# ChrisTho23/DrakeGPT

Measured on NVIDIA B200. Metric: train_tokens_per_sec_TransformerLM_scaled, higher is better.
Workload: dtype bf16

## Files before the change

drakegpt_b200/csrc/attn_tc.cu:

```cuda
#include <cuda.h>
#include <stdlib.h>

#include "common.cuh"
#include "ptx.cuh"

namespace dgpt {

using namespace ptx;

int make_tmap_bf16_2d(CUtensorMap* map, const void* base, int64_t inner, int64_t outer, int64_t ld, int box_outer);

static constexpr int HD = 64;
static constexpr int QT = 128;
static constexpr float kLog2e = 1.4426950408889634f;

struct AttnTcP {
  void *o, *dq, *dk, *dv;
  const void *o_in, *d_o;
  float* lse;
  int64_t o_rs, dq_rs, dk_rs, dv_rs, do_rs;
  int B, NH, T;
  float scale, inv_keep;
  uint32_t thr, site;
  uint64_t seed;
// ... 447 lines not shown
#pragma unroll
      for (int cc = 0; cc < HD; cc += 32) {
        uint32_t r[32];
        tmem_ld32(taddr + nkv * 64 + cc, r);
        tmem_ld_wait();
#pragma unroll
        for (int j = 0; j < 4; ++j) {
          uint4 w;
          w.x = pack_bf16(__uint_as_float(r[8 * j]) * oscale, __uint_as_float(r[8 * j + 1]) * oscale);
          w.y = pack_bf16(__uint_as_float(r[8 * j + 2]) * oscale, __uint_as_float(r[8 * j + 3]) * oscale);
          w.z = pack_bf16(__uint_as_float(r[8 * j + 4]) * oscale, __uint_as_float(r[8 * j + 5]) * oscale);
          w.w = pack_bf16(__uint_as_float(r[8 * j + 6]) * oscale, __uint_as_float(r[8 * j + 7]) * oscale);
          *reinterpret_cast<uint4*>(orow + cc + 8 * j) = w;
        }
      }
      tc_fence_before();
      __syncwarp();
      if (lane == 0) mbar_arrive(&slot_free[g]);
      FTS(5);
    }
  }
  tc_fence_before();
  __syncthreads();
  if (warp == 9) {
    tc_fence_after();
    tmem_dealloc<512>(tmem);
  }
  clock_probe_end(sc.probe);
}

static constexpr int kFwd3Threads = 576;
static constexpr int kFwd3Smem = 2 * kFwd2QK + 2 * 32768 + 4096 + 256 + 1024;

__global__ void __launch_bounds__(kFwd3Threads, 1)
attn_fwd_tc3_kernel(const __grid_constant__ CUtensorMap map_q32, const __grid_constant__ CUtensorMap map_k,
                    const __grid_constant__ CUtensorMap map_v, AttnTcP p, FwdSched sc) {
  extern __shared__ uint8_t smem_raw[];
  uint8_t* smem = reinterpret_cast<uint8_t*>((reinterpret_cast<uintptr_t>(smem_raw) + 1023) & ~(uintptr_t)1023);
  uint8_t* sQK = smem;
  uint8_t* sV = smem + 2 * kFwd2QK;
  float* xch = reinterpret_cast<float*>(sV + 2 * 32768);
  uint64_t* bars = reinterpret_cast<uint64_t*>(sV + 2 * 32768 + 4096);
  uint64_t *qk_full = bars, *qk_empty = bars + 2, *v_full = bars + 4, *v_empty = bars + 6, *s_full = bars + 8,
           *p_full = bars + 10, *o_full = bars + 12, *slot_free = bars + 14;
  uint32_t* tmem_slot = reinterpret_cast<uint32_t*>(bars + 16);

  clock_probe_begin(sc.probe);
  const int warp = threadIdx.x >> 5, lane = threadIdx.x & 31;
  const int ntile = p.T / QT;

  const int G = gridDim.x, c = blockIdx.x;
  const int hq = sc.nheavy / G, hr = sc.nheavy % G;
  const int nh_c = hq + (c < hr ? 1 : 0);
  const int U = (kWHeavy * sc.nheavy + kWLight * sc.nlight + G - 1) / G;
  const int cap_hi = max(0, (U - kWHeavy * (hq + 1)) / kWLight), cap_lo = max(0, (U - kWHeavy * hq) / kWLight);
  const int cap_total = hr * cap_hi + (G - hr) * cap_lo;
  const int l_start = c < hr ? c * cap_hi : hr * cap_hi + (c - hr) * cap_lo;
  const int l0 = min(sc.nlight, l_start), l1 = min(sc.nlight, l_start + (c < hr ? cap_hi : cap_lo));
  const int n_extra = cap_total < sc.nlight ? (sc.nlight - cap_total - c + G - 1) / G : 0;
  const int n_items = nh_c + (l1 - l0) + max(0, n_extra);
  auto item = [&](int n, int& bh, int& qt) {
    if (n < nh_c) {
      bh = c + n * G; qt = ntile - 1;
    } else {
      const int m = n - nh_c;
      bh = m < l1 - l0 ? l0 + m : cap_total + c + (m - (l1 - l0)) * G;
      qt = 0;
    }
  };

  if (threadIdx.x == 0) {
    prefetch_tensormap(&map_q32);
    prefetch_tensormap(&map_k);
    prefetch_tensormap(&map_v);
    for (int g = 0; g < 2; ++g) {
      mbar_init(&qk_full[g], 1);
      mbar_init(&qk_empty[g], 1);
      mbar_init(&v_full[g], 1);
      mbar_init(&v_empty[g], 1);
      mbar_init(&s_full[g], 1);
      mbar_init(&p_full[g], 8);
      mbar_init(&o_full[g], 1);
      mbar_init(&slot_free[g], 8);
    }
    fence_barrier_init();
  }
  if (warp == 17) tmem_alloc<512>(tmem_slot);
  tc_fence_before();
  __syncthreads();
  tc_fence_after();
  const uint32_t tmem = *tmem_slot;
  pdl_grid_sync();

  if (warp == 16) {
    for (int n = 0; n < n_items; ++n) {
      const int g = n & 1, k = n >> 1;
      int bh, qt;
      item(n, bh, qt);
      const int nkv = qt + 1, b = bh / p.NH, h = bh % p.NH, row0 = b * p.T;
      uint8_t* q_s = sQK + g * kFwd2QK;
      uint8_t* v_s = sV + g * 32768;
      mbar_wait(&qk_empty[g], (k & 1) ^ 1);
      if (elect_one()) {
        mbar_expect_tx(&qk_full[g], 16384 * (1 + nkv));
        for (int qb = 0; qb < 4; ++qb)
          tma_load_2d(q_s + qb * 4096, &map_q32, &qk_full[g], h * HD, row0 + qt * QT + (g ? 3 - qb : qb) * 32);
        for (int j = 0; j < nkv; ++j) tma_load_2d(q_s + 16384 * (1 + j), &map_k, &qk_full[g], h * HD, row0 + j * QT);
      }
      __syncwarp();
      mbar_wait(&v_empty[g], (k & 1) ^ 1);
      if (elect_one()) {
        mbar_expect_tx(&v_full[g], 16384 * nkv);
        for (int kb = 0; kb < 2 * nkv; ++kb) tma_load_2d(v_s + kb * 8192, &map_v, &v_full[g], h * HD, row0 + kb * 64);
      }
      __syncwarp();
    }
  } else if (warp == 17) {
    constexpr uint32_t idesc_s = make_idesc_bf16(128, 128, 0, 0);
    constexpr uint32_t idesc_o = make_idesc_bf16(128, 64, 0, 1);
    int next_s = 0, next_pv = 0;
    while (next_pv < n_items) {
      bool progressed = false;
      if (next_s < n_items) {
        const int g = next_s & 1, k = next_s >> 1;
        if (mbar_test(&qk_full[g], k & 1) && mbar_test(&slot_free[g], (k & 1) ^ 1)) {
          tc_fence_after();
          int bh, qt;
          item(next_s, bh, qt);
          const int nkv = qt + 1;
          const uint64_t dq0 = make_smem_desc_sw128(smem_u32(sQK + g * kFwd2QK), 16, 1024);
          const uint64_t dk0 = make_smem_desc_sw128(smem_u32(sQK + g * kFwd2QK + 16384), 16, 1024);
          if (elect_one()) {
            for (int j = 0; j < nkv; ++j) {
#pragma unroll
              for (int kk = 0; kk < 4; ++kk)
                tc_mma_bf16(tmem + g * 256 + j * 128, dq0 + (uint64_t)(kk * 2), dk0 + (uint64_t)(j * 1024 + kk * 2), idesc_s, kk > 0);
            }
            tc_commit(&s_full[g]);
            tc_commit(&qk_empty[g]);
          }
          __syncwarp();
          ++next_s;
          progressed = true;
        }
      }
      if (next_pv < next_s) {
        const int g = next_pv & 1, k = next_pv >> 1;
        if (mbar_test(&p_full[g], k & 1) && mbar_test(&v_full[g], k & 1)) {
          tc_fence_after();
          int bh, qt;
          item(next_pv, bh, qt);
          const int nkv = qt + 1;
          const uint32_t ocol = nkv == 2 ? 192u : 128u;
          const uint64_t dv0 = make_smem_desc_sw128(smem_u32(sV + g * 32768), 8192, 1024);
          if (elect_one()) {
            for (int kb = 0; kb < 2 * nkv; ++kb) {
              const uint32_t pcol = kb < nkv ? (uint32_t)(kb * 32) : (uint32_t)(nkv * 64 + (kb - nkv) * 32);
#pragma unroll
              for (int kk = 0; kk < 4; ++kk)
                tc_mma_bf16_ts(tmem + g * 256 + ocol, tmem + g * 256 + pcol + kk * 8, dv0 + (uint64_t)(kb * 512 + kk * 128), idesc_o,
                               (kb | kk) > 0);
            }
            tc_commit(&o_full[g]);
            tc_commit(&v_empty[g]);
          }
          __syncwarp();
          ++next_pv;
          progressed = true;
        }
      }
      if (!progressed) __nanosleep(32);
    }
  } else {
    const int g = warp >> 3;
    const int quad = warp & 3;
    const int hc = (warp >> 2) & 1;
    const int rblk = g ? 3 - quad : quad;
    const int row = rblk * 32 + lane;
    const uint32_t taddr = tmem + (uint32_t)(g * 256) + ((uint32_t)(quad * 32) << 16);
    float* xmax = xch + g * 512;
    float* xsum = xmax + 256;
    uint64_t seed = p.seed;
    if (p.thr && p.seed_dev) seed += *p.seed_dev;
    const float sc2 = p.scale * kLog2e;
    for (int n = g; n < n_items; n += 2) {
      const int k = n >> 1;
      int bh, qt;
      item(n, bh, qt);
      const int nkv = qt + 1, b = bh / p.NH, h = bh % p.NH, row0 = b * p.T;
      const int qg = qt * QT + row;
      const int hcols = nkv * (QT / 2);
      const int c_beg = hc * hcols, c_end = c_beg + hcols;
      const uint32_t pbase = hc ? (uint32_t)hcols : 0u;
      const uint32_t ocol = nkv == 2 ? 192u : 128u;
#define FTS3(i) do { if (sc.probe && blockIdx.x == 0 && warp == 0 && lane == 0 && k < 3) sc.probe[4 + k * 8 + (i)] = (unsigned long long)clock64(); } while (0)
      FTS3(0);
      mbar_wait(&s_full[g], k & 1);
      FTS3(1);
      tc_fence_after();
      const int qg_max = qt * QT + rblk * 32 + 31, qg_min = qt * QT + rblk * 32;
      float mx = -INFINITY;
      for (int cc = c_beg; cc < c_end && cc <= qg_max; cc += 32) {
        uint32_t r[32];
        tmem_ld32(taddr + cc, r);
        tmem_ld_wait();
        if (cc + 31 <= qg_min) {
#pragma unroll
          for (int j = 0; j < 32; ++j) mx = fmaxf(mx, __uint_as_float(r[j]));
        } else {
#pragma unroll
          for (int j = 0; j < 32; ++j)
            if (cc + j <= qg) mx = fmaxf(mx, __uint_as_float(r[j]));
        }
      }
      xmax[hc * 128 + quad * 32 + lane] = mx;
      asm volatile("bar.sync %0, 256;" ::"r"(2 + g) : "memory");
      mx = fmaxf(mx, xmax[(hc ^ 1) * 128 + quad * 32 + lane]);
      FTS3(2);
      const float msc = mx * sc2;
      float sum = 0.f;
      const uint64_t base = (((uint64_t)b * p.NH + h) * p.T + qg) * (uint64_t)p.T;
      DropGroup dg = {0u, 0u};
      for (int cc = c_beg; cc < c_end; cc += 16) {
        float e[16];
        if (cc > qg_max) {
#pragma unroll
          for (int j = 0; j < 16; ++j) e[j] = 0.f;
        } else {
          uint32_t r[16];
          tmem_ld16(taddr + cc, r);
          tmem_ld_wait();
          if (cc + 15 <= qg_min) {
#pragma unroll
            for (int j = 0; j < 16; ++j) {
              const float v = exp2f(__uint_as_float(r[j]) * sc2 - msc);
              sum += v;
              e[j] = v;
            }
          } else {
#pragma unroll
            for (int j = 0; j < 16; ++j) {
              const float v = (cc + j <= qg) ? exp2f(__uint_as_float(r[j]) * sc2 - msc) : 0.f;
              sum += v;
              e[j] = v;
            }
          }
          if (p.thr) {
            if ((cc & 16) == 0) dg = dropout_group(seed, p.site, (base + cc) >> 5);
            const uint32_t e0 = (uint32_t)(cc & 16);
#pragma unroll
            for (int j = 0; j < 16; ++j)
              if (dropout_word(dg, e0 + j) < p.thr) e[j] = 0.f;
          }
        }
        uint32_t pk[8];
#pragma unroll
        for (int j = 0; j < 8; ++j) pk[j] = pack_bf16(e[2 * j], e[2 * j + 1]);
        tmem_st8(taddr + pbase + (uint32_t)((cc - c_beg) >> 1), pk);
      }
      xsum[hc * 128 + quad * 32 + lane] = sum;
      tmem_st_wait();
      tc_fence_before();
      asm volatile("bar.sync %0, 256;" ::"r"(2 + g) : "memory");
      sum += xsum[(hc ^ 1) * 128 + quad * 32 + lane];
      if (hc == 0 && p.lse) p.lse[((int64_t)b * p.NH + h) * p.T + qg] = mx * p.scale + logf(sum);
      __syncwarp();
      if (lane == 0) mbar_arrive(&p_full[g]);
      FTS3(3);
      mbar_wait(&o_full[g], k & 1);
      FTS3(4);
      tc_fence_after();
      const float oscale = p.inv_keep / sum;
      __nv_bfloat16* orow = reinterpret_cast<__nv_bfloat16*>(p.o) + (int64_t)(row0 + qg) * p.o_rs + h * HD + hc * 32;
      {
        uint32_t r[32];
        tmem_ld32(taddr + ocol + hc * 32, r);
        tmem_ld_wait();
#pragma unroll
        for (int j = 0; j < 4; ++j) {
          uint4 w;
          w.x = pack_bf16(__uint_as_float(r[8 * j]) * oscale, __uint_as_float(r[8 * j + 1]) * oscale);
          w.y = pack_bf16(__uint_as_float(r[8 * j + 2]) * oscale, __uint_as_float(r[8 * j + 3]) * oscale);
          w.z = pack_bf16(__uint_as_float(r[8 * j + 4]) * oscale, __uint_as_float(r[8 * j + 5]) * oscale);
          w.w = pack_bf16(__uint_as_float(r[8 * j + 6]) * oscale, __uint_as_float(r[8 * j + 7]) * oscale);
          *reinterpret_cast<uint4*>(orow + 8 * j) = w;
        }
      }
      tc_fence_before();
      __syncwarp();
      if (lane == 0) mbar_arrive(&slot_free[g]);
      FTS3(5);
    }
  }
  tc_fence_before();
  __syncthreads();
  if (warp == 17) {
    tc_fence_after();
    tmem_dealloc<512>(tmem);
  }
  clock_probe_end(sc.probe);
}

static constexpr int kBwdThreads = 64 + 256;
static constexpr int kBwdSmem = 8 * 16384 + 2 * 32768 + 16384 + 2048 + 1024 + 128;

template <bool DIAG, bool DROP>
__device__ __forceinline__ void bwd_chunk_math(const AttnTcP& p, uint32_t lane_addr_st, uint32_t lane_addr_dp, int row, int k0,
                                               float sc, float lse2, float Dq, uint64_t seed, uint64_t base,
                                               float (&pd)[32], float (&ds)[32]) {
  uint32_t st[32], dp[32];
  tmem_ld32(lane_addr_st + k0, st);
  tmem_ld32(lane_addr_dp + k0, dp);
  tmem_ld_wait();
  DropGroup g = {0u, 0u};
  if (DROP) g = dropout_group(seed, p.site, (base + k0) >> 5);
#pragma unroll
  for (int t = 0; t < 32; ++t) {
    float pv = exp2f(__uint_as_float(st[t]) * sc - lse2);
    if (DIAG) pv = (k0 + t) <= row ? pv : 0.f;
    float dpv = __uint_as_float(dp[t]);
    float pdv = pv;
    if (DROP) {
      const bool keep = dropout_word(g, t) >= p.thr;
      dpv = keep ? dpv * p.inv_keep : 0.f;
      pdv = keep ? pv * p.inv_keep : 0.f;
    }
    pd[t] = pdv;
    ds[t] = pv * (dpv - Dq) * p.scale;
  }
}

template <bool DROP>
__global__ void __launch_bounds__(kBwdThreads, 1)
attn_bwd_tc_kernel(const __grid_constant__ CUtensorMap map_q, const __grid_constant__ CUtensorMap map_k,
                   const __grid_constant__ CUtensorMap map_v, const __grid_constant__ CUtensorMap map_do,
                   const __grid_constant__ CUtensorMap map_o, const __grid_constant__ CUtensorMap map_dq,
                   const __grid_constant__ CUtensorMap map_dk, const __grid_constant__ CUtensorMap map_dv, AttnTcP p) {
  extern __shared__ __align__(1024) uint8_t smem[];
  uint8_t* sQ = smem;
  uint8_t* sK = smem + 2 * 16384;
  uint8_t* sV = smem + 4 * 16384;
  uint8_t* sG = smem + 6 * 16384;
  uint8_t* sPd = smem + 8 * 16384;
  uint8_t* sDs = sPd + 32768;
  uint8_t* sSt = sDs + 32768;
  float* lse_s = reinterpret_cast<float*>(sSt + 16384);
  float* D_s = lse_s + 256;
  uint64_t* bars = reinterpret_cast<uint64_t*>(D_s + 256);
  uint64_t *ld_a = bars, *st_full = bars + 1, *ps_full = bars + 2, *drained = bars + 3, *acc_done = bars + 4;
  uint64_t *ld_b = bars + 5, *ld_c = bars + 6;
  uint64_t* acc_free = bars + 7;
  uint32_t* tmem_slot = reinterpret_cast<uint32_t*>(bars + 8);

  const int warp = threadIdx.x >> 5, lane = threadIdx.x & 31;
#ifdef DGPT_ATTN_TS
#define BTS(i) do { if (blockIdx.x == 0 && blockIdx.y == (gridDim.y / 2) && warp == 2 && lane == 0) g_attn_ts[i] = clock64(); } while (0)
#else
#define BTS(i) do { } while (0)
#endif
  BTS(0);
  const int h = blockIdx.x, b = blockIdx.y;
  const int ntile = p.T / QT;
  const int npair = ntile == 1 ? 1 : 3;
  const int row0 = b * p.T;

  if (threadIdx.x == 0) {
    prefetch_tensormap(&map_q);
    prefetch_tensormap(&map_k);
    prefetch_tensormap(&map_v);
    prefetch_tensormap(&map_do);
    prefetch_tensormap(&map_o);
    mbar_init(ld_a, 1);
    mbar_init(ld_b, 1);
    mbar_init(ld_c, 1);
    mbar_init(st_full, 1);
    mbar_init(ps_full, 8);
    mbar_init(drained, 8);
    mbar_init(acc_done, 1);
    mbar_init(acc_free, 1);
    fence_barrier_init();
  }
  if (warp == 0) {
    __syncwarp();
    pdl_grid_sync();
    if (elect_one()) {
      mbar_expect_tx(ld_a, 16384 * 5);
      tma_load_2d(sG, &map_do, ld_a, h * HD, row0);
      tma_load_2d(sPd, &map_o, ld_a, h * HD, row0);
      tma_load_2d(sQ, &map_q, ld_a, h * HD, row0);
      tma_load_2d(sK, &map_k, ld_a, h * HD, row0);
      tma_load_2d(sV, &map_v, ld_a, h * HD, row0);
      if (ntile > 1) {
        mbar_expect_tx(ld_b, 16384 * 3);
        tma_load_2d(sG + 16384, &map_do, ld_b, h * HD, row0 + QT);
        tma_load_2d(sSt, &map_o, ld_b, h * HD, row0 + QT);
        tma_load_2d(sQ + 16384, &map_q, ld_b, h * HD, row0 + QT);
        mbar_expect_tx(ld_c, 16384 * 2);
        tma_load_2d(sK + 16384, &map_k, ld_c, h * HD, row0 + QT);
        tma_load_2d(sV + 16384, &map_v, ld_c, h * HD, row0 + QT);
      }
    }
  }
  if (warp == 1) tmem_alloc<512>(tmem_slot);
  tc_fence_before();
  __syncthreads();
  tc_fence_after();
  const uint32_t tmem = *tmem_slot;
  constexpr uint32_t TM_ST = 0, TM_DP = 128, TM_DV = 256, TM_DK = 320, TM_DQ = 384;
  if (warp != 0) pdl_grid_sync();

  if (warp == 0) {
  } else if (warp == 1) {
    constexpr uint32_t id_kk = make_idesc_bf16(128, 128, 0, 0);
    constexpr uint32_t id_kmn = make_idesc_bf16(128, 64, 0, 1);
    constexpr uint32_t id_mnmn = make_idesc_bf16(128, 64, 1, 1);
    mbar_wait(ld_a, 0);
    tc_fence_after();
    const uint64_t kQ = make_smem_desc_sw128(smem_u32(sQ), 16, 1024), kK = make_smem_desc_sw128(smem_u32(sK), 16, 1024);
    const uint64_t kV = make_smem_desc_sw128(smem_u32(sV), 16, 1024), kG = make_smem_desc_sw128(smem_u32(sG), 16, 1024);
    const uint64_t kDs = make_smem_desc_sw128(smem_u32(sDs), 16, 1024);
    const uint64_t mQ = make_smem_desc_sw128(smem_u32(sQ), 8192, 1024), mK = make_smem_desc_sw128(smem_u32(sK), 8192, 1024);
    const uint64_t mG = make_smem_desc_sw128(smem_u32(sG), 8192, 1024);
    const uint64_t mPd = make_smem_desc_sw128(smem_u32(sPd), 16384, 1024), mDs = make_smem_desc_sw128(smem_u32(sDs), 16384, 1024);
    auto issue_s_dp = [&](int pr) {
      const int i = pr == 0 ? 0 : 1, j = pr == 2 ? 1 : 0;
      if (elect_one()) {
#pragma unroll
        for (int k = 0; k < 4; ++k)
          tc_mma_bf16(tmem + TM_ST, kQ + (uint64_t)(i * 1024 + k * 2), kK + (uint64_t)(j * 1024 + k * 2), id_kk, k > 0);
#pragma unroll
        for (int k = 0; k < 4; ++k)
          tc_mma_bf16(tmem + TM_DP, kG + (uint64_t)(i * 1024 + k * 2), kV + (uint64_t)(j * 1024 + k * 2), id_kk, k > 0);
        tc_commit(st_full);
      }
      __syncwarp();
    };
    issue_s_dp(0);
    for (int pr = 0; pr < npair; ++pr) {
      const int i = pr == 0 ? 0 : 1, j = pr == 2 ? 1 : 0;
      mbar_wait(ps_full, pr & 1);
      if (pr + 1 < npair) {
        mbar_wait(pr + 1 == 1 ? ld_b : ld_c, 0);
        tc_fence_after();
        issue_s_dp(pr + 1);
      }
      if (pr > 0) mbar_wait(drained, (pr - 1) & 1);
      tc_fence_after();
      const uint32_t acc_vk = (pr == 1) ? 1u : 0u;
      const uint32_t acc_q = (pr == 2) ? 1u : 0u;
      if (elect_one()) {
#pragma unroll
        for (int k = 0; k < 8; ++k)
          tc_mma_bf16(tmem + TM_DV, mPd + (uint64_t)(k * 128), mG + (uint64_t)(i * 1024 + k * 128), id_mnmn, acc_vk | (k > 0));
#pragma unroll
        for (int k = 0; k < 8; ++k)
          tc_mma_bf16(tmem + TM_DK, mDs + (uint64_t)(k * 128), mQ + (uint64_t)(i * 1024 + k * 128), id_mnmn, acc_vk | (k > 0));
#pragma unroll
        for (int k = 0; k < 8; ++k)
          tc_mma_bf16(tmem + TM_DQ, kDs + (uint64_t)((k >> 2) * 1024 + (k & 3) * 2), mK + (uint64_t)(j * 1024 + k * 128), id_kmn,
                      acc_q | (k > 0));
        tc_commit(acc_free);
        if (pr == npair - 1) tc_commit(acc_done);
      }
      __syncwarp();
    }
  } else {
    const int cw = warp - 2;
    const int quad = warp & 3;
    const int half = cw >> 2;
    const int rowl = quad * 32 + lane;
    const int ct = threadIdx.x - 64;
    const uint32_t lane_addr = tmem + ((uint32_t)(quad * 32) << 16);
    uint64_t seed = p.seed;
    if (DROP && p.seed_dev) seed += *p.seed_dev;
    if (ct < p.T) lse_s[ct] = p.lse[((int64_t)b * p.NH + h) * p.T + ct] * kLog2e;
    auto compute_D = [&](int tl, const uint8_t* o_tile) {
      if (ct < QT) {
        const int r = ct;
        const uint8_t* gr = sG + tl * 16384 + r * 128;
        const uint8_t* orow = o_tile + r * 128;
        float acc = 0.f;
#pragma unroll
        for (int c = 0; c < 8; ++c) {
          const int off = (c ^ (r & 7)) << 4;
          const uint4 g = *reinterpret_cast<const uint4*>(gr + off), o = *reinterpret_cast<const uint4*>(orow + off);
          const uint32_t gw[4] = {g.x, g.y, g.z, g.w}, ow[4] = {o.x, o.y, o.z, o.w};
#pragma unroll
          for (int t = 0; t < 4; ++t) {
            const float2 gf = __bfloat1622float2(*reinterpret_cast<const __nv_bfloat162*>(&gw[t]));
            const float2 of = __bfloat1622float2(*reinterpret_cast<const __nv_bfloat162*>(&ow[t]));
            acc = fmaf(gf.x, of.x, acc);
            acc = fmaf(gf.y, of.y, acc);
          }
        }
        D_s[tl * QT + r] = acc;
      }
      asm volatile("bar.sync 1, 256;" ::: "memory");
    };
    BTS(1);
    mbar_wait(ld_a, 0);
    BTS(2);
    compute_D(0, sPd);
    const float sc = p.scale * kLog2e;
    int n_stores = 0;

    auto drain = [&](uint32_t tm_col, const CUtensorMap* map, int tile) {
      uint32_t r[32];
      tmem_ld32(lane_addr + tm_col + half * 32, r);
      if (n_stores > 0) {
        if (ct == 0) bulk_wait_read<0>();
        asm volatile("bar.sync 1, 256;" ::: "memory");
      }
      tmem_ld_wait();
      uint8_t* rp = sSt + rowl * 128;
#pragma unroll
      for (int j = 0; j < 4; ++j) {
        uint4 w;
        w.x = pack_bf16(__uint_as_float(r[8 * j]), __uint_as_float(r[8 * j + 1]));
        w.y = pack_bf16(__uint_as_float(r[8 * j + 2]), __uint_as_float(r[8 * j + 3]));
        w.z = pack_bf16(__uint_as_float(r[8 * j + 4]), __uint_as_float(r[8 * j + 5]));
        w.w = pack_bf16(__uint_as_float(r[8 * j + 6]), __uint_as_float(r[8 * j + 7]));
        *reinterpret_cast<uint4*>(rp + (((half * 4 + j) ^ (rowl & 7)) << 4)) = w;
      }
      fence_proxy_async();
      asm volatile("bar.sync 1, 256;" ::: "memory");
      if (ct == 0) {
        tma_store_2d(map, sSt, h * HD, row0 + tile * QT);
        bulk_commit();
      }
      ++n_stores;
    };

    BTS(3);
    for (int pr = 0; pr < npair; ++pr) {
      const int i = pr == 0 ? 0 : 1, j = pr == 2 ? 1 : 0;
      if (pr == 1) {
        mbar_wait(ld_b, 0);
        compute_D(1, sSt);
      }
      BTS(4 + 4 * pr);
      mbar_wait(st_full, pr & 1);
      BTS(5 + 4 * pr);
      tc_fence_after();
      const int qi = i * QT + rowl;
      const float lse2 = lse_s[qi], Dq = D_s[qi];
      const uint64_t base = (((uint64_t)b * p.NH + h) * p.T + qi) * (uint64_t)p.T + (uint64_t)(j * QT);
      float pd[32], ds[32];
      if (i == j) bwd_chunk_math<true, DROP>(p, lane_addr + TM_ST, lane_addr + TM_DP, rowl, half * 64, sc, lse2, Dq, seed, base, pd, ds);
      else bwd_chunk_math<false, DROP>(p, lane_addr + TM_ST, lane_addr + TM_DP, rowl, half * 64, sc, lse2, Dq, seed, base, pd, ds);
      if (pr > 0) {
        mbar_wait(acc_free, (pr - 1) & 1);
        tc_fence_after();
        if (pr == 1) {
          drain(TM_DQ, &map_dq, 0);
        } else {
          drain(TM_DV, &map_dv, 0);
          drain(TM_DK, &map_dk, 0);
        }
        tc_fence_before();
        __syncwarp();
        if (lane == 0) mbar_arrive(drained);
      }
      BTS(6 + 4 * pr);
      store_row32_sw128(sPd, rowl, half * 64, pd);
      store_row32_sw128(sDs, rowl, half * 64, ds);
      if (i == j) bwd_chunk_math<true, DROP>(p, lane_addr + TM_ST, lane_addr + TM_DP, rowl, half * 64 + 32, sc, lse2, Dq, seed, base, pd, ds);
      else bwd_chunk_math<false, DROP>(p, lane_addr + TM_ST, lane_addr + TM_DP, rowl, half * 64 + 32, sc, lse2, Dq, seed, base, pd, ds);
      store_row32_sw128(sPd, rowl, half * 64 + 32, pd);
      store_row32_sw128(sDs, rowl, half * 64 + 32, ds);
      fence_proxy_async();
      tc_fence_before();
      __syncwarp();
      if (lane == 0) mbar_arrive(ps_full);
      BTS(7 + 4 * pr);
    }
    BTS(16);
    mbar_wait(acc_done, 0);
    BTS(17);
    tc_fence_after();
    const int last = ntile - 1;
    {
      if (n_stores > 0) {
        if (ct == 0) bulk_wait_read<0>();
        asm volatile("bar.sync 1, 256;" ::: "memory");
      }
      uint8_t* tiles[3] = {sPd, sDs, sSt};
      const uint32_t cols[3] = {TM_DV, TM_DK, TM_DQ};
#pragma unroll
      for (int q = 0; q < 3; ++q) {
        uint32_t r[32];
        tmem_ld32(lane_addr + cols[q] + half * 32, r);
        tmem_ld_wait();
        uint8_t* rp = tiles[q] + rowl * 128;
#pragma unroll
        for (int j = 0; j < 4; ++j) {
          uint4 w;
          w.x = pack_bf16(__uint_as_float(r[8 * j]), __uint_as_float(r[8 * j + 1]));
          w.y = pack_bf16(__uint_as_float(r[8 * j + 2]), __uint_as_float(r[8 * j + 3]));
          w.z = pack_bf16(__uint_as_float(r[8 * j + 4]), __uint_as_float(r[8 * j + 5]));
          w.w = pack_bf16(__uint_as_float(r[8 * j + 6]), __uint_as_float(r[8 * j + 7]));
          *reinterpret_cast<uint4*>(rp + (((half * 4 + j) ^ (rowl & 7)) << 4)) = w;
        }
      }
      fence_proxy_async();
      asm volatile("bar.sync 1, 256;" ::: "memory");
      if (ct == 0) {
        tma_store_2d(&map_dv, sPd, h * HD, row0 + last * QT);
        tma_store_2d(&map_dk, sDs, h * HD, row0 + last * QT);
        tma_store_2d(&map_dq, sSt, h * HD, row0 + last * QT);
        bulk_commit();
      }
    }
    if (ct == 0) bulk_wait<0>();
    BTS(18);
  }
  tc_fence_before();
  __syncthreads();
  if (warp == 1) {
    tc_fence_after();
    tmem_dealloc<512>(tmem);
  }
}

bool attn_tc_supported(const dgpt_attn_args* a) {
  if (a->dtype != DGPT_BF16 || a->H != HD || a->Tq != a->Tk) return false;
  if (a->Tk != 128 && a->Tk != 256) return false;
  const int64_t T = a->Tk;
  auto ok = [&](const void* ptr, int64_t bs, int64_t rs) {
    return ptr && ((uintptr_t)ptr & 15) == 0 && rs % 8 == 0 && bs == T * rs;
  };
  if (!ok(a->q, a->q_bs, a->q_rs) || !ok(a->k, a->k_bs, a->k_rs) || !ok(a->v, a->v_bs, a->v_rs) ||
      !ok(a->o, a->o_bs, a->o_rs))
    return false;
  if (a->d_o) {
    if (!ok(a->d_o, a->do_bs, a->do_rs) || !ok(a->dq, a->dq_bs, a->dq_rs) || !ok(a->dk, a->dk_bs, a->dk_rs) ||
        !ok(a->dv, a->dv_bs, a->dv_rs) || !a->lse)
      return false;
  }
  return true;
}

static AttnTcP make_tc_params(const dgpt_attn_args* a) {
  AttnTcP p;
  p.o = a->o; p.dq = a->dq; p.dk = a->dk; p.dv = a->dv; p.o_in = a->o; p.d_o = a->d_o; p.lse = a->lse;
  p.o_rs = a->o_rs; p.dq_rs = a->dq_rs; p.dk_rs = a->dk_rs; p.dv_rs = a->dv_rs; p.do_rs = a->do_rs;
  p.B = a->B; p.NH = a->NH; p.T = a->Tk;
  p.scale = a->scale; p.inv_keep = 1.f / (1.f - a->dropout_p);
  p.thr = dropout_threshold(a->dropout_p); p.site = a->site; p.seed = a->seed; p.seed_dev = a->seed_dev;
  return p;
}

static int attn_fwd_variant() {
  static int v = -1;
  if (v < 0) { const char* e = getenv("DGPT_ATTN_FWD"); v = e ? atoi(e) : 2; }
  return v;
}

int launch_attn_fwd_tc(const dgpt_attn_args* a, cudaStream_t st) {
  CUtensorMap mq, mk, mv;
  const int64_t rows = (int64_t)a->B * a->Tk, cols = (int64_t)a->NH * HD;
  int rc;
  if ((rc = make_tmap_bf16_2d(&mq, a->q, cols, rows, a->q_rs, QT))) return rc;
  if ((rc = make_tmap_bf16_2d(&mk, a->k, cols, rows, a->k_rs, QT))) return rc;
  if ((rc = make_tmap_bf16_2d(&mv, a->v, cols, rows, a->v_rs, 64))) return rc;
  AttnTcP p = make_tc_params(a);
  if (attn_fwd_variant() != 1) {
    if ((rc = make_tmap_bf16_2d(&mq, a->q, cols, rows, a->q_rs, 32))) return rc;
    static bool attr2 = false;
    if (!attr2) {
      cudaError_t e = cudaFuncSetAttribute(attn_fwd_tc2_kernel, cudaFuncAttributeMaxDynamicSharedMemorySize, kFwd2Smem);
      if (e != cudaSuccess) { set_error("attn_fwd_tc2: smem attribute: %s", cudaGetErrorString(e)); return DGPT_E_LAUNCH; }
      attr2 = true;
    }
    const int ntile = a->Tk / QT, bh = a->B * a->NH;
    FwdSched sc;
    sc.nheavy = ntile > 1 ? bh : 0;
    sc.nlight = bh;
    sc.probe = clock_probe_buffer();
    int sms = dgpt_sm_count();
    if (sms <= 0) sms = 148;
    const int grid = min(sms, sc.nheavy + sc.nlight);
    if (attn_fwd_variant() == 3) {
      static bool attr3 = false;
      if (!attr3) {
        cudaError_t e = cudaFuncSetAttribute(attn_fwd_tc3_kernel, cudaFuncAttributeMaxDynamicSharedMemorySize, kFwd3Smem);
        if (e != cudaSuccess) { set_error("attn_fwd_tc3: smem attribute: %s", cudaGetErrorString(e)); return DGPT_E_LAUNCH; }
        attr3 = true;
      }
      launch_pdl(attn_fwd_tc3_kernel, dim3(grid), dim3(kFwd3Threads), kFwd3Smem, st, mq, mk, mv, p, sc);
      return check_launch("attn_fwd_tc3");
    }
    launch_pdl(attn_fwd_tc2_kernel, dim3(grid), dim3(kFwd2Threads), kFwd2Smem, st, mq, mk, mv, p, sc);
    return check_launch("attn_fwd_tc2");
  }
  static bool attr = false;
  if (!attr) {
    cudaError_t e = cudaFuncSetAttribute(attn_fwd_tc_kernel, cudaFuncAttributeMaxDynamicSharedMemorySize, kFwdSmem);
    if (e != cudaSuccess) { set_error("attn_fwd_tc: smem attribute: %s", cudaGetErrorString(e)); return DGPT_E_LAUNCH; }
    attr = true;
  }
  dim3 grid(a->Tk / QT, a->NH, a->B);
  launch_pdl(attn_fwd_tc_kernel, grid, dim3(kFwdThreads), kFwdSmem, st, mq, mk, mv, p);
#ifdef DGPT_ATTN_TS
  {
    cudaStreamSynchronize(st);
    long long h[64];
    cudaMemcpyFromSymbol(h, g_attn_ts, sizeof(h));
    printf("attn fwd CTA(qt=1,h=0,b=B/2): setup %lld | qk load done %lld | S ready %lld | pass1 %lld | pass2 %lld | PV wait %lld | epilogue %lld | exit %lld\n",
           h[1] - h[0], h[8] - h[0], h[2] - h[0], h[3] - h[2], h[4] - h[3], h[5] - h[4], h[6] - h[5], h[7] - h[6]);
    fflush(stdout);
  }
#endif
  return check_launch("attn_fwd_tc");
}

int launch_attn_bwd_tc(const dgpt_attn_args* a, cudaStream_t st) {
  CUtensorMap mq, mk, mv, mg, mo, mdq, mdk, mdv;
  const int64_t rows = (int64_t)a->B * a->Tk, cols = (int64_t)a->NH * HD;
  int rc;
  if ((rc = make_tmap_bf16_2d(&mq, a->q, cols, rows, a->q_rs, QT))) return rc;
  if ((rc = make_tmap_bf16_2d(&mk, a->k, cols, rows, a->k_rs, QT))) return rc;
  if ((rc = make_tmap_bf16_2d(&mv, a->v, cols, rows, a->v_rs, QT))) return rc;
  if ((rc = make_tmap_bf16_2d(&mg, a->d_o, cols, rows, a->do_rs, QT))) return rc;
  if ((rc = make_tmap_bf16_2d(&mo, a->o, cols, rows, a->o_rs, QT))) return rc;
  if ((rc = make_tmap_bf16_2d(&mdq, a->dq, cols, rows, a->dq_rs, QT))) return rc;
  if ((rc = make_tmap_bf16_2d(&mdk, a->dk, cols, rows, a->dk_rs, QT))) return rc;
  if ((rc = make_tmap_bf16_2d(&mdv, a->dv, cols, rows, a->dv_rs, QT))) return rc;
  static bool attr = false;
  if (!attr) {
    cudaError_t e = cudaFuncSetAttribute(attn_bwd_tc_kernel<true>, cudaFuncAttributeMaxDynamicSharedMemorySize, kBwdSmem);
    if (e == cudaSuccess)
      e = cudaFuncSetAttribute(attn_bwd_tc_kernel<false>, cudaFuncAttributeMaxDynamicSharedMemorySize, kBwdSmem);
    if (e != cudaSuccess) { set_error("attn_bwd_tc: smem attribute: %s", cudaGetErrorString(e)); return DGPT_E_LAUNCH; }
    attr = true;
  }
  AttnTcP p = make_tc_params(a);
  dim3 grid(a->NH, a->B);
  if (p.thr) launch_pdl(attn_bwd_tc_kernel<true>, grid, dim3(kBwdThreads), kBwdSmem, st, mq, mk, mv, mg, mo, mdq, mdk, mdv, p);
  else launch_pdl(attn_bwd_tc_kernel<false>, grid, dim3(kBwdThreads), kBwdSmem, st, mq, mk, mv, mg, mo, mdq, mdk, mdv, p);
#ifdef DGPT_ATTN_TS
  {
    cudaStreamSynchronize(st);
    long long h[64];
    cudaMemcpyFromSymbol(h, g_attn_ts, sizeof(h));
    printf("attn bwd CTA: setup %lld | load wait %lld | D %lld |", h[1] - h[0], h[2] - h[1], h[3] - h[2]);
    for (int pr = 0; pr < 3; ++pr)
      printf(" pair%d: S/dP wait %lld, drains %lld, chunks %lld |", pr, h[5 + 4 * pr] - h[4 + 4 * pr], h[6 + 4 * pr] - h[5 + 4 * pr],
             h[7 + 4 * pr] - h[6 + 4 * pr]);
    printf(" acc wait %lld | final drains %lld | total %lld\n", h[17] - h[16], h[18] - h[17], h[18] - h[0]);
    fflush(stdout);
  }
#endif
  return check_launch("attn_bwd_tc");
}

}
```

Before: 7.713 million.

## Make attention backward kernel persistent with pipelined per-head loads and stats

Converts the attention backward kernel from one CTA per (batch, head) to a persistent grid sized to the SM count, where each CTA loops over several (batch, head) items. TMA loads for the next item are gated by new free barriers so they can overlap compute on the current one. The D = rowsum(dO·O) and lse stats are precomputed into a multi-slot ring from global memory instead of TMA-loading O. Drains of the previous pair's accumulators now overlap with the next pair's chunk math. This is meant to remove per-CTA setup, TMEM allocation and load latency, at the cost of more complex barrier phase tracking and less parallelism when there are fewer items than SMs.

```diff
diff --git a/drakegpt_b200/csrc/attn_tc.cu b/drakegpt_b200/csrc/attn_tc.cu
--- a/drakegpt_b200/csrc/attn_tc.cu
+++ b/drakegpt_b200/csrc/attn_tc.cu
@@ -773,7 +773,8 @@
 }
 
 static constexpr int kBwdThreads = 64 + 256;
-static constexpr int kBwdSmem = 8 * 16384 + 2 * 32768 + 16384 + 2048 + 1024 + 128;
+static constexpr int kBwdStatSlots = 4;
+static constexpr int kBwdSmem = 8 * 16384 + 2 * 32768 + 16384 + kBwdStatSlots * 2048 + 1024 + 128;
 
 template <bool DIAG, bool DROP>
 __device__ __forceinline__ void bwd_chunk_math(const AttnTcP& p, uint32_t lane_addr_st, uint32_t lane_addr_dp, int row, int k0,
@@ -801,12 +802,18 @@
   }
 }
 
+#ifdef DGPT_ATTN_TS
+#define BTS(i) do { if (blockIdx.x == 0 && warp == 2 && lane == 0 && (i) < 64) g_attn_ts[i] = clock64(); } while (0)
+#else
+#define BTS(i) do { } while (0)
+#endif
+
 template <bool DROP>
 __global__ void __launch_bounds__(kBwdThreads, 1)
 attn_bwd_tc_kernel(const __grid_constant__ CUtensorMap map_q, const __grid_constant__ CUtensorMap map_k,
                    const __grid_constant__ CUtensorMap map_v, const __grid_constant__ CUtensorMap map_do,
-                   const __grid_constant__ CUtensorMap map_o, const __grid_constant__ CUtensorMap map_dq,
-                   const __grid_constant__ CUtensorMap map_dk, const __grid_constant__ CUtensorMap map_dv, AttnTcP p) {
+                   const __grid_constant__ CUtensorMap map_dq, const __grid_constant__ CUtensorMap map_dk,
+                   const __grid_constant__ CUtensorMap map_dv, AttnTcP p) {
   extern __shared__ __align__(1024) uint8_t smem[];
   uint8_t* sQ = smem;
   uint8_t* sK = smem + 2 * 16384;
@@ -816,61 +823,31 @@
   uint8_t* sDs = sPd + 32768;
   uint8_t* sSt = sDs + 32768;
   float* lse_s = reinterpret_cast<float*>(sSt + 16384);
-  float* D_s = lse_s + 256;
-  uint64_t* bars = reinterpret_cast<uint64_t*>(D_s + 256);
-  uint64_t *ld_a = bars, *st_full = bars + 1, *ps_full = bars + 2, *drained = bars + 3, *acc_done = bars + 4;
-  uint64_t *ld_b = bars + 5, *ld_c = bars + 6;
-  uint64_t* acc_free = bars + 7;
-  uint32_t* tmem_slot = reinterpret_cast<uint32_t*>(bars + 8);
+  float* D_s = lse_s + kBwdStatSlots * 256;
+  uint64_t* bars = reinterpret_cast<uint64_t*>(D_s + kBwdStatSlots * 256);
+  uint64_t *ld_a = bars, *ld_b = bars + 1, *ld_c = bars + 2;
+  uint64_t *free_a = bars + 3, *free_k = bars + 4, *free_b = bars + 5;
+  uint64_t *st_full = bars + 6, *ps_full = bars + 7, *acc_free = bars + 8;
+  uint32_t* tmem_slot = reinterpret_cast<uint32_t*>(bars + 9);
 
   const int warp = threadIdx.x >> 5, lane = threadIdx.x & 31;
-#ifdef DGPT_ATTN_TS
-#define BTS(i) do { if (blockIdx.x == 0 && blockIdx.y == (gridDim.y / 2) && warp == 2 && lane == 0) g_attn_ts[i] = clock64(); } while (0)
-#else
-#define BTS(i) do { } while (0)
-#endif
   BTS(0);
-  const int h = blockIdx.x, b = blockIdx.y;
+  const int G = gridDim.x, c = blockIdx.x;
+  const int n_items = (p.B * p.NH - c + G - 1) / G;
   const int ntile = p.T / QT;
   const int npair = ntile == 1 ? 1 : 3;
-  const int row0 = b * p.T;
+  const int n_pairs = n_items * npair;
 
   if (threadIdx.x == 0) {
     prefetch_tensormap(&map_q);
     prefetch_tensormap(&map_k);
     prefetch_tensormap(&map_v);
     prefetch_tensormap(&map_do);
-    prefetch_tensormap(&map_o);
-    mbar_init(ld_a, 1);
-    mbar_init(ld_b, 1);
-    mbar_init(ld_c, 1);
-    mbar_init(st_full, 1);
-    mbar_init(ps_full, 8);
-    mbar_init(drained, 8);
-    mbar_init(acc_done, 1);
-    mbar_init(acc_free, 1);
+    prefetch_tensormap(&map_dq);
+    prefetch_tensormap(&map_dk);
+    prefetch_tensormap(&map_dv);
+    for (int i = 0; i < 9; ++i) mbar_init(&bars[i], i == 7 ? 8 : 1);
     fence_barrier_init();
-  }
-  if (warp == 0) {
-    __syncwarp();
-    pdl_grid_sync();
-    if (elect_one()) {
-      mbar_expect_tx(ld_a, 16384 * 5);
-      tma_load_2d(sG, &map_do, ld_a, h * HD, row0);
-      tma_load_2d(sPd, &map_o, ld_a, h * HD, row0);
-      tma_load_2d(sQ, &map_q, ld_a, h * HD, row0);
-      tma_load_2d(sK, &map_k, ld_a, h * HD, row0);
-      tma_load_2d(sV, &map_v, ld_a, h * HD, row0);
-      if (ntile > 1) {
-        mbar_expect_tx(ld_b, 16384 * 3);
-        tma_load_2d(sG + 16384, &map_do, ld_b, h * HD, row0 + QT);
-        tma_load_2d(sSt, &map_o, ld_b, h * HD, row0 + QT);
-        tma_load_2d(sQ + 16384, &map_q, ld_b, h * HD, row0 + QT);
-        mbar_expect_tx(ld_c, 16384 * 2);
-        tma_load_2d(sK + 16384, &map_k, ld_c, h * HD, row0 + QT);
-        tma_load_2d(sV + 16384, &map_v, ld_c, h * HD, row0 + QT);
-      }
-    }
   }
   if (warp == 1) tmem_alloc<512>(tmem_slot);
   tc_fence_before();
@@ -878,23 +855,55 @@
   tc_fence_after();
   const uint32_t tmem = *tmem_slot;
   constexpr uint32_t TM_ST = 0, TM_DP = 128, TM_DV = 256, TM_DK = 320, TM_DQ = 384;
-  if (warp != 0) pdl_grid_sync();
+  pdl_grid_sync();
+  BTS(1);
 
   if (warp == 0) {
+    for (int n = 0; n < n_items; ++n) {
+      const int bh = c + n * G, h = bh % p.NH, row0 = (bh / p.NH) * p.T;
+      const uint32_t prev = (uint32_t)(n - 1) & 1;
+      if (n > 0) mbar_wait(free_a, prev);
+      if (elect_one()) {
+        mbar_expect_tx(ld_a, 16384 * 4);
+        tma_load_2d(sG, &map_do, ld_a, h * HD, row0);
+        tma_load_2d(sQ, &map_q, ld_a, h * HD, row0);
+      }
+      __syncwarp();
+      if (n > 0) mbar_wait(free_k, prev);
+      if (elect_one()) {
+        tma_load_2d(sK, &map_k, ld_a, h * HD, row0);
+        tma_load_2d(sV, &map_v, ld_a, h * HD, row0);
+      }
+      __syncwarp();
+      if (ntile > 1) {
+        if (n > 0) mbar_wait(free_b, prev);
+        if (elect_one()) {
+          mbar_expect_tx(ld_b, 16384 * 2);
+          tma_load_2d(sG + 16384, &map_do, ld_b, h * HD, row0 + QT);
+          tma_load_2d(sQ + 16384, &map_q, ld_b, h * HD, row0 + QT);
+          mbar_expect_tx(ld_c, 16384 * 2);
+          tma_load_2d(sK + 16384, &map_k, ld_c, h * HD, row0 + QT);
+          tma_load_2d(sV + 16384, &map_v, ld_c, h * HD, row0 + QT);
+        }
+        __syncwarp();
+      }
+    }
   } else if (warp == 1) {
     constexpr uint32_t id_kk = make_idesc_bf16(128, 128, 0, 0);
     constexpr uint32_t id_kmn = make_idesc_bf16(128, 64, 0, 1);
     constexpr uint32_t id_mnmn = make_idesc_bf16(128, 64, 1, 1);
-    mbar_wait(ld_a, 0);
-    tc_fence_after();
     const uint64_t kQ = make_smem_desc_sw128(smem_u32(sQ), 16, 1024), kK = make_smem_desc_sw128(smem_u32(sK), 16, 1024);
     const uint64_t kV = make_smem_desc_sw128(smem_u32(sV), 16, 1024), kG = make_smem_desc_sw128(smem_u32(sG), 16, 1024);
     const uint64_t kDs = make_smem_desc_sw128(smem_u32(sDs), 16, 1024);
     const uint64_t mQ = make_smem_desc_sw128(smem_u32(sQ), 8192, 1024), mK = make_smem_desc_sw128(smem_u32(sK), 8192, 1024);
     const uint64_t mG = make_smem_desc_sw128(smem_u32(sG), 8192, 1024);
     const uint64_t mPd = make_smem_desc_sw128(smem_u32(sPd), 16384, 1024), mDs = make_smem_desc_sw128(smem_u32(sDs), 16384, 1024);
-    auto issue_s_dp = [&](int pr) {
+    auto loaded = [&](int gp) { return gp % npair == 0 ? ld_a : gp % npair == 1 ? ld_b : ld_c; };
+    auto issue_s_dp = [&](int gp) {
+      const int pr = gp % npair;
       const int i = pr == 0 ? 0 : 1, j = pr == 2 ? 1 : 0;
+      mbar_wait(loaded(gp), (uint32_t)(gp / npair) & 1);
+      tc_fence_after();
       if (elect_one()) {
 #pragma unroll
         for (int k = 0; k < 4; ++k)
@@ -907,15 +916,12 @@
       __syncwarp();
     };
     issue_s_dp(0);
-    for (int pr = 0; pr < npair; ++pr) {
+    for (int gp = 0; gp < n_pairs; ++gp) {
+      const int pr = gp % npair;
       const int i = pr == 0 ? 0 : 1, j = pr == 2 ? 1 : 0;
-      mbar_wait(ps_full, pr & 1);
-      if (pr + 1 < npair) {
-        mbar_wait(pr + 1 == 1 ? ld_b : ld_c, 0);
-        tc_fence_after();
-        issue_s_dp(pr + 1);
-      }
-      if (pr > 0) mbar_wait(drained, (pr - 1) & 1);
+      mbar_wait(ps_full, (uint32_t)gp & 1);
+      const bool next_first = gp + 1 < n_pairs && mbar_test(loaded(gp + 1), (uint32_t)((gp + 1) / npair) & 1);
+      if (next_first) issue_s_dp(gp + 1);
       tc_fence_after();
       const uint32_t acc_vk = (pr == 1) ? 1u : 0u;
       const uint32_t acc_q = (pr == 2) ? 1u : 0u;
@@ -931,9 +937,14 @@
           tc_mma_bf16(tmem + TM_DQ, kDs + (uint64_t)((k >> 2) * 1024 + (k & 3) * 2), mK + (uint64_t)(j * 1024 + k * 128), id_kmn,
                       acc_q | (k > 0));
         tc_commit(acc_free);
-        if (pr == npair - 1) tc_commit(acc_done);
-      }
-      __syncwarp();
+        if (gp + npair < n_pairs) {
+          if (pr == 0) tc_commit(free_a);
+          if (pr == min(1, npair - 1)) tc_commit(free_k);
+          if (pr == 2) tc_commit(free_b);
+        }
+      }
+      __syncwarp();
+      if (!next_first && gp + 1 < n_pairs) issue_s_dp(gp + 1);
     }
   } else {
     const int cw = warp - 2;
@@ -944,18 +955,26 @@
     const uint32_t lane_addr = tmem + ((uint32_t)(quad * 32) << 16);
     uint64_t seed = p.seed;
     if (DROP && p.seed_dev) seed += *p.seed_dev;
-    if (ct < p.T) lse_s[ct] = p.lse[((int64_t)b * p.NH + h) * p.T + ct] * kLog2e;
-    auto compute_D = [&](int tl, const uint8_t* o_tile) {
-      if (ct < QT) {
-        const int r = ct;
-        const uint8_t* gr = sG + tl * 16384 + r * 128;
-        const uint8_t* orow = o_tile + r * 128;
+    const float sc = p.scale * kLog2e;
+    int n_stores = 0;
+
+    auto load_stats = [&](int n) {
+      if (ct < p.T) {
+        const int bh = c + n * G, h = bh % p.NH;
+        const int64_t grow = (int64_t)(bh / p.NH) * p.T + ct;
+        const uint4* gr = reinterpret_cast<const uint4*>(reinterpret_cast<const __nv_bfloat16*>(p.d_o) + grow * p.do_rs + h * HD);
+        const uint4* orow = reinterpret_cast<const uint4*>(reinterpret_cast<const __nv_bfloat16*>(p.o_in) + grow * p.o_rs + h * HD);
+        const float l = p.lse[(int64_t)bh * p.T + ct];
+        uint4 gv[8], ov[8];
+#pragma unroll
+        for (int k = 0; k < 8; ++k) {
+          gv[k] = __ldg(gr + k);
+          ov[k] = __ldg(orow + k);
+        }
         float acc = 0.f;
 #pragma unroll
-        for (int c = 0; c < 8; ++c) {
-          const int off = (c ^ (r & 7)) << 4;
-          const uint4 g = *reinterpret_cast<const uint4*>(gr + off), o = *reinterpret_cast<const uint4*>(orow + off);
-          const uint32_t gw[4] = {g.x, g.y, g.z, g.w}, ow[4] = {o.x, o.y, o.z, o.w};
+        for (int k = 0; k < 8; ++k) {
+          const uint32_t gw[4] = {gv[k].x, gv[k].y, gv[k].z, gv[k].w}, ow[4] = {ov[k].x, ov[k].y, ov[k].z, ov[k].w};
 #pragma unroll
           for (int t = 0; t < 4; ++t) {
             const float2 gf = __bfloat1622float2(*reinterpret_cast<const __nv_bfloat162*>(&gw[t]));
@@ -964,18 +983,12 @@
             acc = fmaf(gf.y, of.y, acc);
           }
         }
-        D_s[tl * QT + r] = acc;
-      }
-      asm volatile("bar.sync 1, 256;" ::: "memory");
+        lse_s[(n % kBwdStatSlots) * 256 + ct] = l * kLog2e;
+        D_s[(n % kBwdStatSlots) * 256 + ct] = acc;
+      }
     };
-    BTS(1);
-    mbar_wait(ld_a, 0);
-    BTS(2);
-    compute_D(0, sPd);
-    const float sc = p.scale * kLog2e;
-    int n_stores = 0;
-
-    auto drain = [&](uint32_t tm_col, const CUtensorMap* map, int tile) {
+
+    auto drain = [&](uint32_t tm_col, const CUtensorMap* map, int bh, int tile) {
       uint32_t r[32];
       tmem_ld32(lane_addr + tm_col + half * 32, r);
       if (n_stores > 0) {
@@ -996,43 +1009,88 @@
       fence_proxy_async();
       asm volatile("bar.sync 1, 256;" ::: "memory");
       if (ct == 0) {
-        tma_store_2d(map, sSt, h * HD, row0 + tile * QT);
+        tma_store_2d(map, sSt, (bh % p.NH) * HD, (bh / p.NH) * p.T + tile * QT);
         bulk_commit();
       }
       ++n_stores;
     };
-
-    BTS(3);
-    for (int pr = 0; pr < npair; ++pr) {
+    auto drain_pair = [&](int n, int pr) {
+      const int bh = c + n * G;
+      if (pr == npair - 1) {
+        drain(TM_DV, &map_dv, bh, ntile - 1);
+        drain(TM_DK, &map_dk, bh, ntile - 1);
+        drain(TM_DQ, &map_dq, bh, ntile - 1);
+      } else if (pr == 0) {
+        drain(TM_DQ, &map_dq, bh, 0);
+      } else {
+        drain(TM_DV, &map_dv, bh, 0);
+        drain(TM_DK, &map_dk, bh, 0);
+      }
+    };
+
+    for (int n = 0; n < n_items && n < kBwdStatSlots; ++n) {
+      const int bh = c + n * G, h = bh % p.NH;
+      const int64_t row_b = (int64_t)(bh / p.NH) * p.T;
+      uint4 gv[8], ov[8];
+#pragma unroll
+      for (int k = 0; k < 8; ++k) {
+        const int r = cw * 32 + 4 * k + (lane >> 3), ch = lane & 7;
+        if (r < p.T) {
+          gv[k] = __ldg(reinterpret_cast<const uint4*>(reinterpret_cast<const __nv_bfloat16*>(p.d_o) + (row_b + r) * p.do_rs + h * HD) + ch);
+          ov[k] = __ldg(reinterpret_cast<const uint4*>(reinterpret_cast<const __nv_bfloat16*>(p.o_in) + (row_b + r) * p.o_rs + h * HD) + ch);
+        }
+      }
+      const float l = ct < p.T ? p.lse[(int64_t)bh * p.T + ct] : 0.f;
+#pragma unroll
+      for (int k = 0; k < 8; ++k) {
+        const int r = cw * 32 + 4 * k + (lane >> 3), ch = lane & 7;
+        if (r < p.T) {
+          *reinterpret_cast<uint4*>(sDs + r * 128 + ((ch ^ (r & 7)) << 4)) = gv[k];
+          *reinterpret_cast<uint4*>(sPd + r * 128 + ((ch ^ (r & 7)) << 4)) = ov[k];
+        }
+      }
+      __syncwarp();
+      if (ct < p.T) {
+        float acc = 0.f;
+#pragma unroll
+        for (int k = 0; k < 8; ++k) {
+          const uint4 g4 = *reinterpret_cast<const uint4*>(sDs + ct * 128 + ((k ^ (ct & 7)) << 4));
+          const uint4 o4 = *reinterpret_cast<const uint4*>(sPd + ct * 128 + ((k ^ (ct & 7)) << 4));
+          const uint32_t gw[4] = {g4.x, g4.y, g4.z, g4.w}, ow[4] = {o4.x, o4.y, o4.z, o4.w};
+#pragma unroll
+          for (int t = 0; t < 4; ++t) {
+            const float2 gf = __bfloat1622float2(*reinterpret_cast<const __nv_bfloat162*>(&gw[t]));
+            const float2 of = __bfloat1622float2(*reinterpret_cast<const __nv_bfloat162*>(&ow[t]));
+            acc = fmaf(gf.x, of.x, acc);
+            acc = fmaf(gf.y, of.y, acc);
+          }
+        }
+        lse_s[(n % kBwdStatSlots) * 256 + ct] = l * kLog2e;
+        D_s[(n % kBwdStatSlots) * 256 + ct] = acc;
+      }
+      __syncwarp();
+    }
+    asm volatile("bar.sync 1, 256;" ::: "memory");
+    for (int gp = 0; gp < n_pairs; ++gp) {
+      const int n = gp / npair, pr = gp % npair;
       const int i = pr == 0 ? 0 : 1, j = pr == 2 ? 1 : 0;
-      if (pr == 1) {
-        mbar_wait(ld_b, 0);
-        compute_D(1, sSt);
-      }
-      BTS(4 + 4 * pr);
-      mbar_wait(st_full, pr & 1);
-      BTS(5 + 4 * pr);
+      const int bh = c + n * G;
+      BTS(gp < 15 ? 2 + 4 * gp : 64);
+      mbar_wait(st_full, (uint32_t)gp & 1);
+      BTS(gp < 15 ? 3 + 4 * gp : 64);
       tc_fence_after();
       const int qi = i * QT + rowl;
-      const float lse2 = lse_s[qi], Dq = D_s[qi];
-      const uint64_t base = (((uint64_t)b * p.NH + h) * p.T + qi) * (uint64_t)p.T + (uint64_t)(j * QT);
+      const float lse2 = lse_s[(n % kBwdStatSlots) * 256 + qi], Dq = D_s[(n % kBwdStatSlots) * 256 + qi];
+      const uint64_t base = ((uint64_t)bh * p.T + qi) * (uint64_t)p.T + (uint64_t)(j * QT);
       float pd[32], ds[32];
       if (i == j) bwd_chunk_math<true, DROP>(p, lane_addr + TM_ST, lane_addr + TM_DP, rowl, half * 64, sc, lse2, Dq, seed, base, pd, ds);
       else bwd_chunk_math<false, DROP>(p, lane_addr + TM_ST, lane_addr + TM_DP, rowl, half * 64, sc, lse2, Dq, seed, base, pd, ds);
-      if (pr > 0) {
-        mbar_wait(acc_free, (pr - 1) & 1);
+      if (gp > 0) {
+        mbar_wait(acc_free, (uint32_t)(gp - 1) & 1);
         tc_fence_after();
-        if (pr == 1) {
-          drain(TM_DQ, &map_dq, 0);
-        } else {
-          drain(TM_DV, &map_dv, 0);
-          drain(TM_DK, &map_dk, 0);
-        }
-        tc_fence_before();
-        __syncwarp();
-        if (lane == 0) mbar_arrive(drained);
-      }
-      BTS(6 + 4 * pr);
+        drain_pair((gp - 1) / npair, (gp - 1) % npair);
+      }
+      BTS(gp < 15 ? 4 + 4 * gp : 64);
       store_row32_sw128(sPd, rowl, half * 64, pd);
       store_row32_sw128(sDs, rowl, half * 64, ds);
       if (i == j) bwd_chunk_math<true, DROP>(p, lane_addr + TM_ST, lane_addr + TM_DP, rowl, half * 64 + 32, sc, lse2, Dq, seed, base, pd, ds);
@@ -1043,47 +1101,18 @@
       tc_fence_before();
       __syncwarp();
       if (lane == 0) mbar_arrive(ps_full);
-      BTS(7 + 4 * pr);
-    }
-    BTS(16);
-    mbar_wait(acc_done, 0);
-    BTS(17);
+      BTS(gp < 15 ? 5 + 4 * gp : 64);
+      if (pr == npair - 1 && n >= 1 && n + kBwdStatSlots - 1 < n_items) {
+        load_stats(n + kBwdStatSlots - 1);
+        asm volatile("bar.sync 1, 256;" ::: "memory");
+      }
+    }
+    mbar_wait(acc_free, (uint32_t)(n_pairs - 1) & 1);
+    BTS(62);
     tc_fence_after();
-    const int last = ntile - 1;
-    {
-      if (n_stores > 0) {
-        if (ct == 0) bulk_wait_read<0>();
-        asm volatile("bar.sync 1, 256;" ::: "memory");
-      }
-      uint8_t* tiles[3] = {sPd, sDs, sSt};
-      const uint32_t cols[3] = {TM_DV, TM_DK, TM_DQ};
-#pragma unroll
-      for (int q = 0; q < 3; ++q) {
-        uint32_t r[32];
-        tmem_ld32(lane_addr + cols[q] + half * 32, r);
-        tmem_ld_wait();
-        uint8_t* rp = tiles[q] + rowl * 128;
-#pragma unroll
-        for (int j = 0; j < 4; ++j) {
-          uint4 w;
-          w.x = pack_bf16(__uint_as_float(r[8 * j]), __uint_as_float(r[8 * j + 1]));
-          w.y = pack_bf16(__uint_as_float(r[8 * j + 2]), __uint_as_float(r[8 * j + 3]));
-          w.z = pack_bf16(__uint_as_float(r[8 * j + 4]), __uint_as_float(r[8 * j + 5]));
-          w.w = pack_bf16(__uint_as_float(r[8 * j + 6]), __uint_as_float(r[8 * j + 7]));
-          *reinterpret_cast<uint4*>(rp + (((half * 4 + j) ^ (rowl & 7)) << 4)) = w;
-        }
-      }
-      fence_proxy_async();
-      asm volatile("bar.sync 1, 256;" ::: "memory");
-      if (ct == 0) {
-        tma_store_2d(&map_dv, sPd, h * HD, row0 + last * QT);
-        tma_store_2d(&map_dk, sDs, h * HD, row0 + last * QT);
-        tma_store_2d(&map_dq, sSt, h * HD, row0 + last * QT);
-        bulk_commit();
-      }
-    }
+    drain_pair(n_items - 1, npair - 1);
     if (ct == 0) bulk_wait<0>();
-    BTS(18);
+    BTS(63);
   }
   tc_fence_before();
   __syncthreads();
@@ -1186,14 +1215,13 @@
 }
 
 int launch_attn_bwd_tc(const dgpt_attn_args* a, cudaStream_t st) {
-  CUtensorMap mq, mk, mv, mg, mo, mdq, mdk, mdv;
+  CUtensorMap mq, mk, mv, mg, mdq, mdk, mdv;
   const int64_t rows = (int64_t)a->B * a->Tk, cols = (int64_t)a->NH * HD;
   int rc;
   if ((rc = make_tmap_bf16_2d(&mq, a->q, cols, rows, a->q_rs, QT))) return rc;
   if ((rc = make_tmap_bf16_2d(&mk, a->k, cols, rows, a->k_rs, QT))) return rc;
   if ((rc = make_tmap_bf16_2d(&mv, a->v, cols, rows, a->v_rs, QT))) return rc;
   if ((rc = make_tmap_bf16_2d(&mg, a->d_o, cols, rows, a->do_rs, QT))) return rc;
-  if ((rc = make_tmap_bf16_2d(&mo, a->o, cols, rows, a->o_rs, QT))) return rc;
   if ((rc = make_tmap_bf16_2d(&mdq, a->dq, cols, rows, a->dq_rs, QT))) return rc;
   if ((rc = make_tmap_bf16_2d(&mdk, a->dk, cols, rows, a->dk_rs, QT))) return rc;
   if ((rc = make_tmap_bf16_2d(&mdv, a->dv, cols, rows, a->dv_rs, QT))) return rc;
@@ -1206,19 +1234,24 @@
     attr = true;
   }
   AttnTcP p = make_tc_params(a);
-  dim3 grid(a->NH, a->B);
-  if (p.thr) launch_pdl(attn_bwd_tc_kernel<true>, grid, dim3(kBwdThreads), kBwdSmem, st, mq, mk, mv, mg, mo, mdq, mdk, mdv, p);
-  else launch_pdl(attn_bwd_tc_kernel<false>, grid, dim3(kBwdThreads), kBwdSmem, st, mq, mk, mv, mg, mo, mdq, mdk, mdv, p);
+  int sms = dgpt_sm_count();
+  if (sms <= 0) sms = 148;
+  const int grid = min(sms, a->B * a->NH);
+  if (p.thr) launch_pdl(attn_bwd_tc_kernel<true>, dim3(grid), dim3(kBwdThreads), kBwdSmem, st, mq, mk, mv, mg, mdq, mdk, mdv, p);
+  else launch_pdl(attn_bwd_tc_kernel<false>, dim3(grid), dim3(kBwdThreads), kBwdSmem, st, mq, mk, mv, mg, mdq, mdk, mdv, p);
 #ifdef DGPT_ATTN_TS
   {
     cudaStreamSynchronize(st);
     long long h[64];
     cudaMemcpyFromSymbol(h, g_attn_ts, sizeof(h));
-    printf("attn bwd CTA: setup %lld | load wait %lld | D %lld |", h[1] - h[0], h[2] - h[1], h[3] - h[2]);
-    for (int pr = 0; pr < 3; ++pr)
-      printf(" pair%d: S/dP wait %lld, drains %lld, chunks %lld |", pr, h[5 + 4 * pr] - h[4 + 4 * pr], h[6 + 4 * pr] - h[5 + 4 * pr],
-             h[7 + 4 * pr] - h[6 + 4 * pr]);
-    printf(" acc wait %lld | final drains %lld | total %lld\n", h[17] - h[16], h[18] - h[17], h[18] - h[0]);
+    const int npair = a->Tk / QT == 1 ? 1 : 3, n_pairs = min(15, (a->B * a->NH + grid - 1) / grid * npair);
+    printf("attn bwd CTA 0 (%d items): setup %lld |", n_pairs / npair, h[1] - h[0]);
+    for (int gp = 0; gp < n_pairs; ++gp) {
+      const long long* t = h + 2 + 4 * gp;
+      printf(" item%d pair%d: S/dP wait %lld, chunk0 + drains %lld, chunk1 %lld, stats %lld |", gp / npair, gp % npair, t[1] - t[0],
+             t[2] - t[1], t[3] - t[2], (gp + 1 < n_pairs ? t[4] : h[62]) - t[3]);
+    }
+    printf(" last drains %lld | total %lld\n", h[63] - h[62], h[63] - h[0]);
     fflush(stdout);
   }
 #endif
```

Result: no change. 7.770 million, median of 6 (+0.7%).
